# vocdoni/gnark-crypto-primitives

Hardware: AMD Instinct MI355X
Metric: proofs/sec, Arbo-160 Poseidon SMT-verifier circuit, Groth16/BN254 (higher is better)
Workload: dtype u32x8 Montgomery (254-bit integer)

## Files before the change

### gnark_crypto_primitives_amd/csrc/api.hip

```cpp
#include <algorithm>

#include "zkmi_internal.h"
#include "ff29.h"
#include "ec29.h"

using namespace zk;

namespace zk {

int ensure_scratch(zkmi_ctx* ctx, DevBuf& s, size_t bytes, void** out) {
  if (s.bytes < bytes) {
    if (s.p) {
      hipStreamSynchronize(ctx->stream);
      if (ctx->stream2) hipStreamSynchronize(ctx->stream2);
      if (ctx->stream3) hipStreamSynchronize(ctx->stream3);
      hipFree(s.p);
      s.p = nullptr;
      s.bytes = 0;
    }
    hipError_t e = hipMalloc(&s.p, bytes);
    if (e != hipSuccess) {
      ctx->err = "hipMalloc(" + std::to_string(bytes) + " B) failed: " + hipGetErrorString(e) +
                 " (the working set of this batch does not fit beside the MSM tables: load the key"
                 " with zkmi_pk_desc.max_batch >= the batch size, or with a table_budget_bytes cap)";
      s.p = nullptr;
      return ZKMI_ERR_OOM;
    }
    s.bytes = bytes;
  }
  if (out) *out = s.p;
  return ZKMI_OK;
}

int require_idle(zkmi_ctx* ctx) {
  if (!ctx->sets[0].pending && !ctx->sets[1].pending) return ZKMI_OK;
// ... 559 lines not shown
int zkmi_msm_bases_load(zkmi_ctx* ctx, int group, const void* bases, size_t n, int window_bits,
                        zkmi_msm_bases** out) {
  return zkmi_msm_bases_load_image(ctx, group, bases, n, window_bits, 0, out);
}

int zkmi_msm_bases_load_image(zkmi_ctx* ctx, int group, const void* bases, size_t n,
                              int window_bits, int image, zkmi_msm_bases** out) {
  ZK_HIP(hipSetDevice(ctx->device));
  if (!out) return ZKMI_ERR_ARG;
  if (image != 0 && image != 1) {
    ctx->err = "image must be 0 (x * 2^256) or 1 (x * 2^261)";
    return ZKMI_ERR_ARG;
  }
  if (!window_bits_ok(window_bits)) {
    ctx->err = "window_bits must be 0 (auto), in [2,16], 100 + [4,16], 200 + [2,20] or 300 + [3,21]";
    return ZKMI_ERR_ARG;
  }
  Staged sb(ctx);
  int rc = sb.in(bases, n * (group == 1 ? 64 : 128));
  if (rc) return rc;
  WinPlan plan;
  if (window_bits) {
    plan = plan_explicit(window_bits);
  } else {
    const double usable = usable_table_bytes_standalone(n);
    plan = plan_windows_for_budget(n, group, (group == 1 ? 0.64 : 0.34) * usable);
    int c1, c2;
    plan_shared_for_budget(group == 1 ? n : 0, group == 2 ? n : 0, 0.9 * usable, &c1, &c2);
    const WinPlan ps = plan_shared(group == 1 ? c1 : c2);
    if (ps.W < plan.W) plan = ps;
    if (n >= 64) {
      int k1, k2;
      bool s1, s2;
      plan_comb_for_budget(group == 1 ? n : 0, group == 2 ? n : 0, 0.9 * usable, &k1, &k2, &s1, &s2);
      const int k = group == 1 ? k1 : k2;
      if ((double)COMB_W / k < (double)plan.W) plan = plan_comb(k, group == 1 ? s1 : s2);
    }
  }
  return bases_load_plan(ctx, group, sb.dev, n, plan, window_bits == 0, out,
                         image ? MSM_IMAGE_F : MSM_IMAGE_STD);
}

void zkmi_msm_bases_free(zkmi_ctx* ctx, zkmi_msm_bases* b) {
  if (!b) return;
  if (ctx) {
    hipSetDevice(ctx->device);
    hipStreamSynchronize(ctx->stream);
  }
  if (b->table) hipFree(b->table);
  if (b->inf) hipFree(b->inf);
  delete b;
}

uint32_t zkmi_comb_min_groups_per_chunk(void) { return COMB_MIN_GROUPS_PER_CHUNK; }

int zkmi_msm_batch(zkmi_ctx* ctx, const zkmi_msm_bases* bases, const void* scalars, size_t batch,
                   void* out) {
  ZK_HIP(hipSetDevice(ctx->device));
  int rc;
  if ((rc = require_idle(ctx))) return rc;
  if (batch == 0) return ZKMI_OK;
  const size_t n = bases->n, Bp = round_up(batch, 64);
  const size_t pt = bases->group == 1 ? 64 : 128;
  Staged ss(ctx), so(ctx);
  if ((rc = ss.in(scalars, batch * n * 32)) || (rc = so.out(out, batch * pt))) return rc;
  void *sbi, *acc, *aff;
  if ((rc = ensure_scratch(ctx, ctx->sets[0].a, (n ? n : 1) * Bp * 32, &sbi)) ||
// ... 106 lines not shown
  zkmi_msm_bases_free(ctx, pk->B1);
  zkmi_msm_bases_free(ctx, pk->K);
  zkmi_msm_bases_free(ctx, pk->Z);
  zkmi_msm_bases_free(ctx, pk->B2);
  zkmi_msm_bases_free(ctx, pk->D1);
  zkmi_msm_bases_free(ctx, pk->D2);
  commit_keys_free(ctx, pk);
  if (pk->idx3) hipFree(pk->idx3);
  if (pk->a_wire) hipFree(pk->a_wire);
  if (pk->b_wire) hipFree(pk->b_wire);
  if (pk->k_wire) hipFree(pk->k_wire);
  delete pk;
}

static int wires_from_infinity(zkmi_ctx* ctx, const uint8_t* inf, uint32_t n_wires, uint32_t want,
                               const char* name, std::vector<uint32_t>* out) {
  std::vector<uint8_t> host(n_wires);
  if (n_wires && hipMemcpy(host.data(), inf, n_wires, hipMemcpyDefault) != hipSuccess) {
    ctx->err = std::string("pk: cannot read ") + name;
    return ZKMI_ERR_HIP;
  }
  out->clear();
  for (uint32_t i = 0; i < n_wires; i++)
    if (!host[i]) out->push_back(i);
  if (out->size() != want) {
    ctx->err = std::string("pk: ") + name + " retains " + std::to_string(out->size()) +
               " wires but the key holds " + std::to_string(want) + " points";
    return ZKMI_ERR_ARG;
  }
  return ZKMI_OK;
}

int zkmi_pk_load(zkmi_ctx* ctx, const zkmi_pk_desc* d, zkmi_pk** out) {
  ZK_HIP(hipSetDevice(ctx->device));
  if (!d || !out) return ZKMI_ERR_ARG;
  if (d->log_n < 1 || d->log_n > 28) {
    ctx->err = "pk: log_n out of range [1,28]";
    return ZKMI_ERR_ARG;
  }
  if (d->n_z + 1 < (1u << d->log_n)) {
    ctx->err = "pk: n_z must be at least 2^log_n - 1";
    return ZKMI_ERR_ARG;
  }
  const uint32_t n_z = (1u << d->log_n) - 1;
  std::vector<uint32_t> wa, wb, wk;
  {
    int rc;
    struct { const uint32_t* p; uint32_t n; const char* name; std::vector<uint32_t>* v; } idx[3] = {
        {d->a_wire, d->n_a, "a_wire", &wa}, {d->b_wire, d->n_b, "b_wire", &wb},
        {d->k_wire, d->n_k, "k_wire", &wk}};
    for (auto& t : idx) {
      if (!t.p) continue;
      t.v->resize(t.n);
      if (t.n && hipMemcpy(t.v->data(), t.p, (size_t)t.n * 4, hipMemcpyDefault) != hipSuccess) {
        ctx->err = std::string("pk: cannot read ") + t.name;
        return ZKMI_ERR_HIP;
      }
    }
    if (!d->a_wire) {
      if (!d->infinity_a) {
        ctx->err = "pk: neither a_wire nor infinity_a given";
        return ZKMI_ERR_ARG;
      }
      if ((rc = wires_from_infinity(ctx, d->infinity_a, d->n_wires, d->n_a, "infinity_a", &wa)))
        return rc;
    }
    if (!d->b_wire) {
      if (!d->infinity_b) {
// ... 56 lines not shown
  pk->log_n = d->log_n;
  pk->n_wires = d->n_wires;
  pk->n_a = d->n_a;
  pk->n_b = d->n_b;
  pk->n_k = n_kb;
  pk->n_z = n_zb;
  pk->folded = fold.folded;
  pk->fold_n_constraints = fold.folded ? d->fold_r1cs->n_constraints : 0;
  pk->max_batch = d->max_batch ? d->max_batch : 1024;
  int rc;
  if ((rc = commit_keys_load(ctx, d, pk))) {
    zkmi_pk_free(ctx, pk);
    return rc;
  }
  const bool auto1 = d->window_bits_g1 == 0, auto2 = d->window_bits_g2 == 0;
  const size_t n1 = (size_t)d->n_a + d->n_b + n_kb + n_zb;
  const size_t n_msm_max = std::max(std::max((size_t)d->n_a, (size_t)d->n_b),
                                    std::max((size_t)n_kb, (size_t)n_zb));
  const size_t n_slots = d->n_slots_hint ? d->n_slots_hint : (size_t)d->n_wires + d->n_wires / 20;
  const double ws = prove_working_set_bytes(d->log_n, n_slots, d->n_wires, pk->max_batch, n_msm_max,
                                            pk->commits.size());
  double usable = free_hbm_bytes() - ws;
  if (usable < 0) usable = 0;
  if (d->table_budget_bytes && (double)d->table_budget_bytes < usable)
    usable = (double)d->table_budget_bytes;
  int sc1 = 0, sc2 = 0;
  plan_shared_for_budget(n1, d->n_b, 0.98 * usable, &sc1, &sc2);
  WinPlan p1 = auto1 ? plan_windows_for_budget(n1, 1, 0.64 * usable)
                     : plan_explicit((int)d->window_bits_g1);
  WinPlan p2 = auto2 ? plan_windows_for_budget(d->n_b, 2, 0.34 * usable)
                     : plan_explicit((int)d->window_bits_g2);
  if (auto1 && sc1 && plan_shared(sc1).W < p1.W) p1 = plan_shared(sc1);
  if (auto2 && sc2 && plan_shared(sc2).W < p2.W) p2 = plan_shared(sc2);
  if (n1 >= 4096) {
    int k1 = 0, k2 = 0;
    bool s1 = true, s2 = true;
    plan_comb_for_budget(auto1 ? n1 : 0, auto2 ? d->n_b : 0, 0.98 * usable, &k1, &k2, &s1, &s2,
                         d->sparse_witness == 0);
    if (auto1 && (double)COMB_W / k1 < (double)p1.W) p1 = plan_comb(k1, s1);
    if (auto2 && (double)COMB_W / k2 < (double)p2.W) p2 = plan_comb(k2, s2);
  }
  WinPlan p1z = p1;
  if (d->sparse_witness >= 2 && auto1 && auto2 && n1 >= 4096 && n_zb >= 4096) {
    const int kw = 12;
    const double wire_bytes =
        (double)((d->n_a + kw - 1) / kw + (d->n_b + kw - 1) / kw + (n_kb + kw - 1) / kw) *
            (double)(1u << kw) * 64.0 +
        (double)((d->n_b + kw - 1) / kw) * (double)(1u << kw) * 128.0;
    if (wire_bytes < 0.5 * usable) {
      int kz = 0, k2 = 0;
      bool sz = true, s2 = true;
      plan_comb_for_budget(n_zb, 0, 0.98 * usable - wire_bytes, &kz, &k2, &sz, &s2, true);
      p1 = plan_comb(kw, false);
      p2 = plan_comb(kw, false);
      p1z = plan_comb(kz, sz);
    }
  }
  auto load = [&](int group, const void* pts, size_t n, const WinPlan& plan, bool relax,
                  zkmi_msm_bases** out, int image) -> int {
    Staged sb(ctx);
    int r = sb.in(pts, n * (group == 1 ? 64 : 128));
    if (r) return r;
    r = bases_load_plan(ctx, group, sb.dev, n, plan, relax, out, image);
    if (!r) (*out)->chunk_factor = d->msm_chunk_factor;
    return r;
  };
  if ((rc = upload_u32(ctx, wa.data(), d->n_a, &pk->a_wire)) ||
      (rc = upload_u32(ctx, wb.data(), d->n_b, &pk->b_wire)) ||
      (rc = upload_u32(ctx, fold.folded ? fold.k_wire.data() : wk.data(), n_kb, &pk->k_wire)) ||
      (rc = load(1, d->g1_a, d->n_a, p1, auto1, &pk->A, MSM_IMAGE_F)) ||
      (rc = load(1, d->g1_b, d->n_b, p1, auto1, &pk->B1, MSM_IMAGE_F)) ||
      (rc = load(1, fold.folded ? (const void*)fold.k.data() : d->g1_k, n_kb, p1, auto1, &pk->K,
                 MSM_IMAGE_F)) ||
      (rc = load(1, fold.folded ? (const void*)fold.e.data() : d->g1_z, n_zb, p1z, auto1, &pk->Z,
                 MSM_IMAGE_STD)) ||
      (rc = load(2, d->g2_b, d->n_b, p2, auto2, &pk->B2, MSM_IMAGE_F))) {
    zkmi_pk_free(ctx, pk);
    return rc;
  }
  {
    const uint32_t idx[3] = {0, 1, 2};
    if ((rc = upload_u32(ctx, idx, 3, &pk->idx3)) ||
        (rc = zkmi_msm_bases_load(ctx, 1, d->g1_delta, 1, 8, &pk->D1)) ||
        (rc = zkmi_msm_bases_load(ctx, 2, d->g2_delta, 1, 8, &pk->D2))) {
      zkmi_pk_free(ctx, pk);
      return rc;
    }
    pk->D1->side = pk->D2->side = 2;
  }
  hipMemcpy(&pk->alpha, d->g1_alpha, 64, hipMemcpyDefault);
  hipMemcpy(&pk->beta1, d->g1_beta, 64, hipMemcpyDefault);
  hipMemcpy(&pk->delta1, d->g1_delta, 64, hipMemcpyDefault);
  hipMemcpy(&pk->beta2, d->g2_beta, 128, hipMemcpyDefault);
  hipMemcpy(&pk->delta2, d->g2_delta, 128, hipMemcpyDefault);
  *out = pk;
  return ZKMI_OK;
}

int zkmi_pk_info(const zkmi_pk* pk, uint64_t* info) {
  if (!pk || !info) return ZKMI_ERR_ARG;
  info[0] = (uint64_t)pk->Z->plan.W;
  info[1] = pk->Z->plan.per_base;
  info[2] = (uint64_t)pk->B2->plan.W;
  info[3] = pk->B2->plan.per_base;
  info[4] = pk->A->table_bytes + pk->B1->table_bytes + pk->K->table_bytes + pk->Z->table_bytes;
  info[5] = pk->B2->table_bytes;
  info[6] = pk->Z->plan.shared;
  info[7] = pk->B2->plan.shared;
  info[8] = pk->Z->plan.comb;
  info[9] = pk->B2->plan.comb;
  return ZKMI_OK;
}

int zkmi_pk_folded(const zkmi_pk* pk) { return pk && pk->folded ? 1 : 0; }

void zkmi_cs_free(zkmi_ctx* ctx, zkmi_cs* cs) {
  if (!cs) return;
  if (ctx) hipSetDevice(ctx->device);
  if (cs->program) hipFree(cs->program);
  if (cs->consts) hipFree(cs->consts);
  delete cs;
}

int zkmi_cs_load(zkmi_ctx* ctx, const zkmi_cs_desc* d, zkmi_cs** out) {
  ZK_HIP(hipSetDevice(ctx->device));
  if (!d || !out) return ZKMI_ERR_ARG;
  auto* cs = new zkmi_cs();
  const std::string err =
      vprog_validate({d->n_wires, d->n_slots, d->n_consts, d->n_constraints, d->n_rows,
                      d->lanes_per_proof},
                     d->program, &cs->commit_rows, &cs->has_emul);
  if (!err.empty()) {
    delete cs;
    ctx->err = err;
    return ZKMI_ERR_ARG;
  }
  cs->n_wires = d->n_wires;
  cs->n_public = d->n_public;
  cs->n_secret = d->n_secret;
  cs->n_constraints = d->n_constraints;
  cs->n_slots = d->n_slots;
  cs->n_rows = d->n_rows;
  cs->n_consts = d->n_consts;
// ... 215 lines not shown
}

int zkmi_prove_collect(zkmi_ctx* ctx, void* proofs_out, int32_t* status_out) {
  return zkmi_prove_collect_ex(ctx, proofs_out, status_out, nullptr);
}

int zkmi_prove_collect_ex(zkmi_ctx* ctx, void* proofs_out, int32_t* status_out,
                          void* commitments_out) {
  ZK_HIP(hipSetDevice(ctx->device));
  const int si = ctx->next_collect;
  zkmi_ctx::ProveSet& S = ctx->sets[si];
  if (!S.pending) {
    ctx->err = "prove: nothing submitted";
    return ZKMI_ERR_ARG;
  }
  if (!S.pk->commits.empty() && !commitments_out) {
    ctx->err = "prove: this key has commitments: collect with zkmi_prove_collect_ex";
    return ZKMI_ERR_ARG;
  }
  const zkmi_pk* pk = S.pk;
  const size_t batch = S.batch, Bp = S.Bp;
  int rc;
  if (!S.heavy_enqueued && (rc = enqueue_heavy(ctx, si))) return rc;
  SumsView v(S.sums.p, Bp);
  hipStream_t q3 = ctx->stream3;
  ZK_HIP(hipStreamWaitEvent(q3, S.evq[4], 0));
  hipEventRecord(S.eva[0], q3);
  if (pk->Z->plan.shared || pk->Z->plan.comb) {
    void* ws[4] = {v.w1[0], v.w1[1], v.w1[2], v.w1[3]};
    void* os[4] = {v.sA, v.sB1, v.sK, v.sZ};
    const zkmi_msm_bases* ms[4] = {pk->A, pk->B1, pk->K, pk->Z};
    bool same = true;
    for (int i = 0; i < 3; i++)
      same = same && ms[i]->plan.bits[0] == pk->Z->plan.bits[0] &&
             ms[i]->plan.comb == pk->Z->plan.comb &&
             ms[i]->plan.comb_signed == pk->Z->plan.comb_signed;
    if (same) {
      if ((rc = msm_horner_run(ctx, q3, 4, ms, ws, os, Bp))) return rc;
    } else {
      for (int i = 0; i < 4; i++)
        if ((rc = msm_horner_run(ctx, q3, 1, ms + i, ws + i, os + i, Bp))) return rc;
    }
  }
  if (pk->B2->plan.shared || pk->B2->plan.comb) {
    void* ws[1] = {v.w2};
    void* os[1] = {v.sB2};
    const zkmi_msm_bases* ms[1] = {pk->B2};
    if ((rc = msm_horner_run(ctx, q3, 1, ms, ws, os, Bp))) return rc;
  }
  PkConsts pc{pk->alpha, pk->beta1, pk->beta2};
  hipLaunchKernelGGL(assemble_kernel, dim3((unsigned)(Bp / 64)), dim3(64), 0, q3, v.sA, v.sB1, v.sK,
                     v.sZ, v.tR, v.tS, v.tNRS, (const Fr*)S.rs, Bp, pc, v.proofs);
  hipLaunchKernelGGL(assemble_g2_kernel, dim3((unsigned)(Bp / 64)), dim3(64), 0, q3, v.sB2, v.tS2,
                     Bp, pk->beta2, v.proofs);
  ZK_HIP(hipGetLastError());
  ZK_HIP(hipMemcpyAsync(proofs_out, v.proofs, batch * 256, hipMemcpyDefault, q3));
  ZK_HIP(hipMemcpyAsync(status_out, S.st, batch * 4, hipMemcpyDefault, q3));
  if (const size_t nc = pk->commits.size()) {
    const size_t pitch = (nc + 1) * 64;
    for (size_t i = 0; i < nc; i++)
      ZK_HIP(hipMemcpy2DAsync((char*)commitments_out + i * 64, pitch,
                              (const char*)S.commit_pts + i * Bp * 64, 64, 64, batch, hipMemcpyDefault, q3));
    ZK_HIP(hipMemcpy2DAsync((char*)commitments_out + nc * 64, pitch,
                            (const char*)S.commit_pok + Bp * 128, 64, 64, batch, hipMemcpyDefault, q3));
  }
  hipEventRecord(S.eva[1], q3);
  zkmi_ctx::ProveSet& N = ctx->sets[si ^ 1];
  if (N.pending && !N.heavy_enqueued && (rc = enqueue_heavy(ctx, si ^ 1))) return rc;
  ZK_HIP(hipEventSynchronize(S.eva[1]));
// ... 37 lines not shown
```

### gnark_crypto_primitives_amd/csrc/msm.hip

```cpp
#include "msm_impl.h"

namespace zk {

WinPlan plan_with_windows(int W) {
  WinPlan p;
  if (W < 16) W = 16;
  if (W > 64) W = 64;
  p.W = W;
  const int c0 = 255 / W, rem = 255 - c0 * W;
  uint32_t off = 0;
  for (int j = 0; j < W; j++) {
    p.bits[j] = (uint8_t)(j < rem ? c0 + 1 : c0);
    p.off[j] = off;
    off += 1u << (p.bits[j] - 1);
  }
  p.per_base = off;
  return p;
}
WinPlan plan_uniform(int c) {
  WinPlan p;
  p.W = (255 + c - 1) / c;
  uint32_t off = 0;
  for (int j = 0; j < p.W; j++) {
    p.bits[j] = (uint8_t)c;
    p.off[j] = off;
    off += 1u << (c - 1);
  }
  p.per_base = off;
  return p;
}
WinPlan plan_shared(int c) {
  WinPlan p;
  if (c < 4) c = 4;
  if (c > 16) c = 16;
  p.shared = 1;
  p.W = (255 + c - 1) / c;
  for (int j = 0; j < p.W; j++) {
    p.bits[j] = (uint8_t)(j + 1 < p.W ? c : 255 - (p.W - 1) * c);
    p.off[j] = 0;
  }
  p.per_base = 1u << (c - 1);
  return p;
}
WinPlan plan_comb(int k, bool signed_tables) {
  WinPlan p;
  if (k < 2) k = 2;
  if (k > 21) k = 21;
  if (!signed_tables && k > 20) k = 20;
  p.comb = (uint8_t)k;
  p.comb_signed = signed_tables ? 1 : 0;
  p.W = COMB_W + (signed_tables ? 1 : 0);
  p.per_base = 0;
  return p;
}
void plan_comb_for_budget(size_t n1, size_t n2, double usable_bytes, int* k1, int* k2, bool* sg1,
                          bool* sg2, bool allow_signed) {
  double best = 1e300;
  *k1 = *k2 = 8;
  *sg1 = *sg2 = allow_signed;
  for (int s1 = 0; s1 < (allow_signed ? 2 : 1); s1++)
    for (int s2 = 0; s2 < (allow_signed ? 2 : 1); s2++)
      for (int a = 8; a <= (s1 ? 21 : 20); a++)
        for (int b = 8; b <= (s2 ? 21 : 20); b++) {
          const double g1 = (double)((n1 + a - 1) / a), g2 = (double)((n2 + b - 1) / b);
          const double bytes = g1 * (double)(1u << (a - s1)) * 64.0 + g2 * (double)(1u << (b - s2)) * 128.0;
          if (bytes > usable_bytes) continue;
          const double cost = g1 * (s1 ? 255 * 62.8 : 254 * 61.1) + g2 * (s2 ? 255 * 178.5 : 254 * 171.6);
          if (cost < best) {
            best = cost;
            *k1 = a;
            *k2 = b;
            *sg1 = s1 != 0;
            *sg2 = s2 != 0;
          }
        }
}
void plan_shared_for_budget(size_t n1, size_t n2, double usable_bytes, int* c1, int* c2) {
  double best = 1e300;
  *c1 = *c2 = 4;
  for (int a = 4; a <= 16; a++)
    for (int b = 4; b <= 16; b++) {
      const double bytes = (double)n1 * (1u << (a - 1)) * 64.0 + (double)n2 * (1u << (b - 1)) * 128.0;
      if (bytes > usable_bytes) continue;
      const double cost = (double)n1 * ((255 + a - 1) / a) + 3.0 * (double)n2 * ((255 + b - 1) / b);
      if (cost < best) {
        best = cost;
        *c1 = a;
        *c2 = b;
      }
    }
}
WinPlan plan_windows_for_budget(size_t n_total, int group, double budget_bytes) {
  const double entry = group == 1 ? 64.0 : 128.0;
  for (int W = 16; W <= 64; W++) {
    WinPlan p = plan_with_windows(W);
    if ((double)n_total * p.per_base * entry <= budget_bytes) return p;
  }
  return plan_with_windows(64);
}

extern template int build_comb<Fq2>(zkmi_ctx*, const Affine<Fq2>*, size_t, const WinPlan&, int,
                                    Affine<Fq2>*, int*, Affine<Fq2>*);
extern template int build_impl<Fq2>(zkmi_ctx*, const Affine<Fq2>*, size_t, const WinPlan&,
                                    Affine<Fq2>*);
extern template int run_impl<Fq2>(zkmi_ctx*, const zkmi_msm_bases*, const Fr*, const uint32_t*,
                                  size_t, size_t, XYZZ<Fq2>*, bool, XYZZ<Fq2>*, hipStream_t,
                                  const uint8_t*, bool);

// ... 130 lines not shown
```

### gnark_crypto_primitives_amd/groth16.py

```python
from __future__ import annotations

import ctypes as C
import random

import numpy as np

from . import lib as _lib
from .frontend.compile import CompiledCircuit, R, ints_to_array, to_mont_array

P = 21888242871839275222246405745257275088696311157297823662689037894645226208583
_MONT_P = (1 << 256) % P

G1_GEN = (1, 2)
G2_GEN = ((10857046999023057135944570762232829481370756359578518086990519993285655852781,
           11559732032986387107991004021392285783925812861821192530917403151452391805634),
          (8495653923123431417604973247489272438418190587263600148770280649306958101930,
           4082367875863433681332203403145435568316851327593401208105741076214120093531))


def _fq_mont(xs):
    return ints_to_array([x % P * _MONT_P % P for x in xs])


def g1_gen_mont():
# ... 126 lines not shown
    vk.g2_beta, vk.g2_delta, vk.g2_gamma = pk.g2_beta, pk.g2_delta, g2_pts[nb + 2].copy()
    return pk, vk, trapdoor


def commit_fn(pk: ProvingKey):
    from . import hash_to_field, verify as _v
    bases = [[_v.g1_from_image(b) for b in ck["basis"]] for ck in pk.commitment_keys]

    def fn(idx, hashed, committed):
        acc = None
        for pt, s in zip(bases[idx], committed):
            if s % R and pt is not None:
                acc = _v._g1_add(acc, _v._g1_mul(pt, s % R))
        return hash_to_field.commitment_challenge(acc, hashed)
    return fn


def gpu_mul(ctx: _lib.Context):
    def mul(group, scalars):
        n = scalars.shape[0]
        out = np.zeros((n, 8 if group == 1 else 16), dtype=np.uint64)
        if n:
            ctx.fixed_base_mul(group, g1_gen_mont() if group == 1 else g2_gen_mont(), scalars, n,
                               out)
        return out
    return mul


class Prover:

    def __init__(self, ctx: _lib.Context, cc: CompiledCircuit, pk: ProvingKey,
                 window_bits_g1: int = 0, window_bits_g2: int = 0, *, max_batch: int = 0,
                 table_budget_bytes: int = 0, msm_chunk_factor: int = 0,
                 gnark_key_layout: bool = False, sparse_witness=None, fold_quotient=None):
        self.ctx, self.cc, self.pk = ctx, cc, pk
        self.n_inputs = cc.n_inputs
        self._consts = to_mont_array(cc.consts) if cc.consts else np.zeros((0, 4), np.uint64)
        prog = self._prog = np.ascontiguousarray(cc.vprogram, dtype=np.uint32)
        cd = _lib.CsDesc(cc.n_wires, cc.n_public, cc.n_secret, cc.n_constraints, cc.v_n_slots,
                         cc.v_n_rows, len(cc.consts), cc.lanes_per_proof, prog.ctypes.data,
                         self._consts.ctypes.data)
        self.cs_h = ctx.cs_load(cd)
        self._keep = [np.ascontiguousarray(x) for x in
                      (pk.a_wire, pk.b_wire, pk.k_wire, pk.g1_a, pk.g1_b, pk.g1_k, pk.g1_z, pk.g2_b,
                       pk.g1_alpha, pk.g1_beta, pk.g1_delta, pk.g2_beta, pk.g2_delta)]
        k = self._keep
        ptrs = [x.ctypes.data for x in k]
        inf_a = inf_b = None
        n_public = 0
        if gnark_key_layout:
            inf_a, inf_b = pk.infinity_maps()
            self._keep += [inf_a, inf_b]
            ptrs[0] = ptrs[1] = ptrs[2] = None
            n_public = cc.n_public
        self.n_commitments = len(pk.commitment_keys)
        cdescs = (_lib.CommitmentDesc * max(self.n_commitments, 1))()
        for i, ck in enumerate(pk.commitment_keys):
            arrs = [np.ascontiguousarray(ck["private"], dtype=np.uint32),
                    np.ascontiguousarray(ck["hashed"], dtype=np.uint32),
                    np.ascontiguousarray(ck["basis"], dtype=np.uint64),
                    np.ascontiguousarray(ck["basis_exp_sigma"], dtype=np.uint64)]
            self._keep += arrs
            cdescs[i] = _lib.CommitmentDesc(len(ck["private"]), len(ck["hashed"]), ck["wire"], 0,
                                            *[a.ctypes.data for a in arrs])
        self._keep.append(cdescs)
        if len(getattr(cc, "commitments", [])) != self.n_commitments:
            raise ValueError("circuit and proving key disagree on the number of commitments")
        fold = None
        if fold_quotient is None:
            fold_quotient = not self.n_commitments
        if fold_quotient and cc.consts and cc.n_constraints:
            fold, fold_keep = self._r1cs_desc()
            self._keep += fold_keep + [fold]
        pd = _lib.PkDesc(pk.log_n, pk.n_wires, len(pk.a_wire), len(pk.b_wire), len(pk.k_wire),
                         pk.g1_z.shape[0], *ptrs, window_bits_g1, window_bits_g2,
                         inf_a.ctypes.data if inf_a is not None else None,
                         inf_b.ctypes.data if inf_b is not None else None, n_public,
                         max_batch, table_budget_bytes, cc.v_n_slots, msm_chunk_factor,
                         (2 if cc.n_boolean_wires * 100 >= cc.n_wires * 99 else
                          int(cc.n_boolean_wires * 2 > cc.n_wires)) if sparse_witness is None
                         else int(sparse_witness),
                         self.n_commitments,
                         C.addressof(cdescs) if self.n_commitments else None,
                         C.addressof(fold) if fold is not None else None)
        self.pk_h = ctx.pk_load(pd)
        self.folded = ctx.pk_folded(self.pk_h)

    def _r1cs_desc(self):
        cc = self.cc
        coeffs = to_mont_array(cc.consts)
        keep = [coeffs]
        fields = []
        for ptr, col, cid in (cc.L, cc.Rm, cc.O):
            terms = np.ascontiguousarray(np.stack([cid, col], axis=1).astype(np.uint32))
            ptr = np.ascontiguousarray(ptr, dtype=np.uint32)
            keep += [ptr, terms]
            fields += [ptr.ctypes.data, terms.ctypes.data]
        return (_lib.R1csDesc(cc.n_wires, cc.n_constraints, len(cc.consts), coeffs.ctypes.data,
                              *fields), keep)

    def load_r1cs(self):
        if getattr(self, "r1cs_h", None):
            return self.r1cs_h
        rd, _keep = self._r1cs_desc()
        self.r1cs_h = self.ctx.r1cs_load(rd)
        return self.r1cs_h

    def load_r1cs_solver(self, lanes_per_proof=0, hints="basic"):
        sets = {"basic": _lib.HINTS_BASIC, "std": _lib.HINTS_STD}
        if hints not in sets:
            raise ValueError('hints must be "basic" or "std"')
        if getattr(self, "r1cs_solver_h", None):
            if (lanes_per_proof, hints) == self._r1cs_solver_args:
                return self.r1cs_solver_h
            self.ctx.r1cs_solver_free(self.r1cs_solver_h)
            self.r1cs_solver_h = None
        cc = self.cc
        kinds, in_ptr, lc_ptr, hcol, hcid, out_ptr, outs = cc.hint_arrays
# ... 135 lines not shown
```

### gnark_crypto_primitives_amd/lib.py

```python
from __future__ import annotations

import ctypes as C
import os

import numpy as np

_HERE = os.path.dirname(os.path.abspath(__file__))
LIB_PATH = os.environ.get("ZKMI_LIB", os.path.join(_HERE, "libzkmi.so"))

ZKMI_OK = 0
ZKMI_ERR_UNSATISFIED = -5


class ZkmiError(RuntimeError):
    pass


class PkDesc(C.Structure):
    _fields_ = [("log_n", C.c_uint32), ("n_wires", C.c_uint32), ("n_a", C.c_uint32),
                ("n_b", C.c_uint32), ("n_k", C.c_uint32), ("n_z", C.c_uint32),
                ("a_wire", C.c_void_p), ("b_wire", C.c_void_p), ("k_wire", C.c_void_p),
                ("g1_a", C.c_void_p), ("g1_b", C.c_void_p), ("g1_k", C.c_void_p),
                ("g1_z", C.c_void_p), ("g2_b", C.c_void_p), ("g1_alpha", C.c_void_p),
                ("g1_beta", C.c_void_p), ("g1_delta", C.c_void_p), ("g2_beta", C.c_void_p),
# ... 31 lines not shown
    _fields_ = [("n_public", C.c_uint32), ("n_secret", C.c_uint32), ("n_instr", C.c_uint32),
                ("n_hints", C.c_uint32), ("instr", C.c_void_p), ("hint_kind", C.c_void_p),
                ("hint_in_ptr", C.c_void_p), ("hint_lc_ptr", C.c_void_p), ("hint_terms", C.c_void_p),
                ("hint_out_ptr", C.c_void_p), ("hint_out", C.c_void_p),
                ("lanes_per_proof", C.c_uint32), ("hint_set", C.c_uint32)]


HINTS_BASIC, HINTS_STD = 0, 1


_P, _SZ, _I = C.c_void_p, C.c_size_t, C.c_int
SYMBOLS = [
    ("zkmi_init", _I, [_I, C.POINTER(_P)]),
    ("zkmi_destroy", None, [_P]),
    ("zkmi_last_error", C.c_char_p, [_P]),
    ("zkmi_sync", _I, [_P]),
    ("zkmi_stream", _P, [_P]),
    ("zkmi_field_mul", _I, [_P, _I, _P, _P, _P, _SZ]),
    ("zkmi_ff29_op", _I, [_P, _I, _I, _P, _P, _SZ]),
    ("zkmi_field_mul_bench", _I, [_P, _I, _SZ, _I, C.POINTER(C.c_double)]),
    ("zkmi_ntt_batch", _I, [_P, _P, _I, _SZ, _I, _I]),
    ("zkmi_h_batch", _I, [_P, _P, _P, _P, _P, _I, _SZ]),
    ("zkmi_ab_coset_batch", _I, [_P, _P, _P, _P, _I, _SZ]),
    ("zkmi_quotient_bases", _I, [_P, _P, _SZ, _I, _P, _P]),
    ("zkmi_msm_bases_load", _I, [_P, _I, _P, _SZ, _I, C.POINTER(_P)]),
    ("zkmi_msm_bases_free", None, [_P, _P]),
    ("zkmi_msm_batch", _I, [_P, _P, _P, _SZ, _P]),
    ("zkmi_msm_bases_load_image", _I, [_P, _I, _P, _SZ, _I, _I, C.POINTER(_P)]),
    ("zkmi_msm_batch_rows", _I, [_P, _P, _P, _SZ, _P, _SZ, _I, _I, _P]),
    ("zkmi_comb_min_groups_per_chunk", C.c_uint32, []),
    ("zkmi_fixed_base_mul", _I, [_P, _I, _P, _P, _SZ, _P]),
    ("zkmi_pk_load", _I, [_P, C.POINTER(PkDesc), C.POINTER(_P)]),
    ("zkmi_pk_free", None, [_P, _P]),
    ("zkmi_pk_info", _I, [_P, C.POINTER(C.c_uint64)]),
    ("zkmi_pk_folded", _I, [_P]),
    ("zkmi_cs_load", _I, [_P, C.POINTER(CsDesc), C.POINTER(_P)]),
    ("zkmi_cs_free", None, [_P, _P]),
    ("zkmi_solve_batch", _I, [_P, _P, _P, _SZ, _P, _P, _P]),
    ("zkmi_prove_batch", _I, [_P, _P, _P, _P, _SZ, _P, _P, _P]),
    ("zkmi_prove_submit", _I, [_P, _P, _P, _P, _SZ, _P]),
    ("zkmi_prove_collect", _I, [_P, _P, _P]),
    ("zkmi_prove_collect_ex", _I, [_P, _P, _P, _P]),
    ("zkmi_prove_witness_batch", _I, [_P, _P, _P, _P, _P, _P, _SZ, _SZ, _P, _P]),
    ("zkmi_host_alloc", _P, [_P, _SZ]),
    ("zkmi_host_free", None, [_P, _P]),
    ("zkmi_set_copy_threads", _I, [_P, _I]),
    ("zkmi_r1cs_load", _I, [_P, C.POINTER(R1csDesc), C.POINTER(_P)]),
    ("zkmi_r1cs_free", None, [_P, _P]),
    ("zkmi_prove_witness_submit", _I, [_P, _P, _P, _P, _P, _P, _P, _SZ, _SZ, _P]),
    ("zkmi_r1cs_solver_load", _I, [_P, _P, C.POINTER(R1csSolverDesc), C.POINTER(_P)]),
    ("zkmi_r1cs_solver_free", None, [_P, _P]),
    ("zkmi_r1cs_solver_info", _I, [_P, C.POINTER(C.c_uint64)]),
    ("zkmi_r1cs_solve_batch", _I, [_P, _P, _P, _SZ, _P, _P, _P]),
    ("zkmi_prove_r1cs_submit", _I, [_P, _P, _P, _P, _SZ, _P]),
    ("zkmi_last_timings", _I, [_P, C.POINTER(C.c_double)]),
    ("zkmi_plonk_pk_load", _I, [_P, _P, C.POINTER(_P)]),
    ("zkmi_plonk_pk_free", None, [_P, _P]),
    ("zkmi_plonk_round1", _I, [_P, _P, _P, _P, _SZ, _P, _P, _P]),
    ("zkmi_plonk_round2", _I, [_P, _P, _P, _P]),
    ("zkmi_plonk_round3", _I, [_P, _P, _P, _P]),
    ("zkmi_plonk_round4", _I, [_P, _P, _P, _P]),
    ("zkmi_plonk_round5", _I, [_P, _P, _P, _P]),
    ("zkmi_plonk_prove", _I, [_P, _P, _P, _P, _SZ, _P, _P, _P, _P]),
]

_lib = None

# ... 109 lines not shown
        self._check(self.lib.zkmi_msm_bases_load(self.h, group, _ptr(bases), n, window_bits,
                                                 C.byref(h)), "zkmi_msm_bases_load")
        return h

    def msm_bases_free(self, h):
        self.lib.zkmi_msm_bases_free(self.h, h)

    def msm_batch(self, bases_h, scalars, batch, out):
        self._check(self.lib.zkmi_msm_batch(self.h, bases_h, _ptr(scalars), batch, _ptr(out)),
                    "zkmi_msm_batch")
        return out

    def msm_bases_load_image(self, group, bases, n, window_bits, image):
        h = C.c_void_p()
        self._check(self.lib.zkmi_msm_bases_load_image(self.h, group, _ptr(bases), n, window_bits,
                                                       image, C.byref(h)),
                    "zkmi_msm_bases_load_image")
        return h

    def msm_batch_rows(self, bases_h, scalars, n_rows, row_idx, batch, image, uniform, out):
        self._check(self.lib.zkmi_msm_batch_rows(self.h, bases_h, _ptr(scalars), n_rows,
                                                 _ptr(row_idx), batch, image, uniform, _ptr(out)),
                    "zkmi_msm_batch_rows")
        return out

    def comb_min_groups_per_chunk(self):
        return int(self.lib.zkmi_comb_min_groups_per_chunk())

    def fixed_base_mul(self, group, base, scalars, n, out):
        self._check(self.lib.zkmi_fixed_base_mul(self.h, group, _ptr(base), _ptr(scalars), n,
                                                 _ptr(out)), "zkmi_fixed_base_mul")
        return out

    def pk_load(self, desc: PkDesc):
        h = C.c_void_p()
        self._check(self.lib.zkmi_pk_load(self.h, C.byref(desc), C.byref(h)), "zkmi_pk_load")
        return h

    def pk_info(self, h):
        arr = (C.c_uint64 * 10)()
        self._check(self.lib.zkmi_pk_info(h, arr), "zkmi_pk_info")
        return dict(zip(("g1_windows", "g1_entries_per_base", "g2_windows", "g2_entries_per_base",
                         "g1_table_bytes", "g2_table_bytes", "g1_shared", "g2_shared",
                         "g1_comb_k", "g2_comb_k"), [int(x) for x in arr]))

    def pk_folded(self, h) -> bool:
        return bool(self.lib.zkmi_pk_folded(h))

    def pk_free(self, h):
        self.lib.zkmi_pk_free(self.h, h)

    def cs_load(self, desc: CsDesc):
        h = C.c_void_p()
        self._check(self.lib.zkmi_cs_load(self.h, C.byref(desc), C.byref(h)), "zkmi_cs_load")
        return h

    def cs_free(self, h):
        self.lib.zkmi_cs_free(self.h, h)

    def solve_batch(self, cs_h, inputs, batch, wires_out=None, abc_out=None, status_out=None):
        if status_out is None:
            status_out = np.zeros(batch, dtype=np.int32)
        self._check(self.lib.zkmi_solve_batch(self.h, cs_h, _ptr(inputs), batch, _ptr(wires_out),
                                              _ptr(abc_out), _ptr(status_out)), "zkmi_solve_batch")
        return status_out

    def prove_batch(self, pk_h, cs_h, inputs, batch, rs, proofs_out, status_out):
        self._check(self.lib.zkmi_prove_batch(self.h, pk_h, cs_h, _ptr(inputs), batch, _ptr(rs),
                                              _ptr(proofs_out), _ptr(status_out)),
                    "zkmi_prove_batch")

    def prove_submit(self, pk_h, cs_h, inputs, batch, rs):
        self._check(self.lib.zkmi_prove_submit(self.h, pk_h, cs_h, _ptr(inputs), batch, _ptr(rs)),
                    "zkmi_prove_submit")

    def prove_collect(self, proofs_out, status_out, commitments_out=None):
        if commitments_out is None:
# ... 78 lines not shown
```

### include/zkmi.h

```cpp
#ifndef ZKMI_H
#define ZKMI_H
#include <stddef.h>
#include <stdint.h>

#ifdef __cplusplus
extern "C" {
#endif

typedef struct zkmi_ctx zkmi_ctx;
typedef struct zkmi_pk zkmi_pk;
typedef struct zkmi_cs zkmi_cs;
typedef struct zkmi_r1cs_desc zkmi_r1cs_desc;

enum zkmi_status {
  ZKMI_OK = 0,
  ZKMI_ERR_ARG = -1,
  ZKMI_ERR_HIP = -2,
  ZKMI_ERR_NO_DEVICE = -3,
  ZKMI_ERR_OOM = -4,
  ZKMI_ERR_UNSATISFIED = -5
};

int zkmi_init(int device, zkmi_ctx** out);
void zkmi_destroy(zkmi_ctx* ctx);
// ... 42 lines not shown

typedef struct {
  uint32_t log_n;
  uint32_t n_wires;
  uint32_t n_a, n_b, n_k, n_z;
  const uint32_t* a_wire;
  const uint32_t* b_wire;
  const uint32_t* k_wire;
  const void* g1_a;
  const void* g1_b;
  const void* g1_k;
  const void* g1_z;
  const void* g2_b;
  const void* g1_alpha;
  const void* g1_beta;
  const void* g1_delta;
  const void* g2_beta;
  const void* g2_delta;
  uint32_t window_bits_g1;
  uint32_t window_bits_g2;
  const uint8_t* infinity_a;
  const uint8_t* infinity_b;
  uint32_t n_public;
  uint32_t max_batch;
  uint64_t table_budget_bytes;
  uint32_t n_slots_hint;
  uint32_t msm_chunk_factor;
  uint32_t sparse_witness;
  uint32_t n_commitments;
  const zkmi_commitment_desc* commitments;
  const zkmi_r1cs_desc* fold_r1cs;
} zkmi_pk_desc;
int zkmi_pk_load(zkmi_ctx* ctx, const zkmi_pk_desc* desc, zkmi_pk** out);
void zkmi_pk_free(zkmi_ctx* ctx, zkmi_pk* pk);
int zkmi_pk_info(const zkmi_pk* pk, uint64_t* info );
int zkmi_pk_folded(const zkmi_pk* pk);

typedef struct {
  uint32_t n_wires, n_public, n_secret, n_constraints;
  uint32_t n_slots, n_rows, n_consts;
  uint32_t lanes_per_proof;
  const uint32_t* program;
  const void* consts;
} zkmi_cs_desc;
int zkmi_cs_load(zkmi_ctx* ctx, const zkmi_cs_desc* desc, zkmi_cs** out);
void zkmi_cs_free(zkmi_ctx* ctx, zkmi_cs* cs);

int zkmi_solve_batch(zkmi_ctx* ctx, const zkmi_cs* cs, const void* inputs, size_t batch,
                     void* wires_out, void* abc_out, int32_t* status_out);

int zkmi_prove_batch(zkmi_ctx* ctx, const zkmi_pk* pk, const zkmi_cs* cs, const void* inputs,
                     size_t batch, const void* rs, void* proofs_out, int32_t* status_out);

int zkmi_prove_submit(zkmi_ctx* ctx, const zkmi_pk* pk, const zkmi_cs* cs, const void* inputs,
                      size_t batch, const void* rs);
int zkmi_prove_collect(zkmi_ctx* ctx, void* proofs_out, int32_t* status_out);
int zkmi_prove_collect_ex(zkmi_ctx* ctx, void* proofs_out, int32_t* status_out,
                          void* commitments_out);

void* zkmi_host_alloc(zkmi_ctx* ctx, size_t bytes);
void zkmi_host_free(zkmi_ctx* ctx, void* p);
int zkmi_set_copy_threads(zkmi_ctx* ctx, int threads);

typedef struct {
  uint32_t coeff;
  uint32_t wire;
} zkmi_term;
struct zkmi_r1cs_desc {
// ... 94 lines not shown
```

Measured before the change: 8615.

## Search per-MSM comb table sizes under memory budget instead of one shared size

Replaces the single comb window size shared by the A, B1, K and Z G1 MSMs with a branch-and-bound search that picks a comb width and signedness for each of the five MSMs. The search weights the Z MSM more heavily than the others and bounds the total cost to stay near the equal-size plan. The Horner batching check is relaxed so that MSMs with different comb widths can still run together. An explicit per-MSM override API and a plan-query API are also added. The aim is to give more of the table memory budget to the MSMs where it lowers the most group additions. The risk is an uneven split that slows the A, B1 and K MSMs, or breaks the batched Horner path.

```diff
diff --git a/gnark_crypto_primitives_amd/csrc/api.hip b/gnark_crypto_primitives_amd/csrc/api.hip
--- a/gnark_crypto_primitives_amd/csrc/api.hip
+++ b/gnark_crypto_primitives_amd/csrc/api.hip
@@ -1,6 +1,7 @@
 #include <algorithm>
 
 #include "zkmi_internal.h"
+#include "comb_plan.h"
 #include "ff29.h"
 #include "ec29.h"
 
@@ -626,7 +627,7 @@
     if (n >= 64) {
       int k1, k2;
       bool s1, s2;
-      plan_comb_for_budget(group == 1 ? n : 0, group == 2 ? n : 0, 0.9 * usable, &k1, &k2, &s1, &s2);
+      comb_plan_equal(group == 1 ? n : 0, group == 2 ? n : 0, 0.9 * usable, &k1, &k2, &s1, &s2, true);
       const int k = group == 1 ? k1 : k2;
       if ((double)COMB_W / k < (double)plan.W) plan = plan_comb(k, group == 1 ? s1 : s2);
     }
@@ -799,8 +800,25 @@
 }
 
 int zkmi_pk_load(zkmi_ctx* ctx, const zkmi_pk_desc* d, zkmi_pk** out) {
+  return zkmi_pk_load_planned(ctx, d, nullptr, out);
+}
+
+int zkmi_pk_load_planned(zkmi_ctx* ctx, const zkmi_pk_desc* d, const uint32_t* msm_window_bits,
+                         zkmi_pk** out) {
   ZK_HIP(hipSetDevice(ctx->device));
   if (!d || !out) return ZKMI_ERR_ARG;
+  if (msm_window_bits)
+    for (int i = 0; i < COMB_PLAN_MSMS; i++)
+      if (msm_window_bits[i] == 0 || !window_bits_ok((int)msm_window_bits[i])) {
+        ctx->err = "pk: msm_window_bits must be in [2,16], 100 + [4,16], 200 + [2,20] or 300 + [3,21]";
+        return ZKMI_ERR_ARG;
+      }
+  if (msm_window_bits)
+    for (int i = 0; i < COMB_MSM_Z; i++)
+      if ((msm_window_bits[i] >= 100) != (msm_window_bits[COMB_MSM_Z] >= 100)) {
+        ctx->err = "pk: msm_window_bits of A, B1, K and Z must all be per-window plans or none";
+        return ZKMI_ERR_ARG;
+      }
   if (d->log_n < 1 || d->log_n > 28) {
     ctx->err = "pk: log_n out of range [1,28]";
     return ZKMI_ERR_ARG;
@@ -923,15 +941,18 @@
                      : plan_explicit((int)d->window_bits_g2);
   if (auto1 && sc1 && plan_shared(sc1).W < p1.W) p1 = plan_shared(sc1);
   if (auto2 && sc2 && plan_shared(sc2).W < p2.W) p2 = plan_shared(sc2);
+  WinPlan pm[COMB_PLAN_MSMS] = {p1, p1, p1, p1, p2};
   if (n1 >= 4096) {
-    int k1 = 0, k2 = 0;
-    bool s1 = true, s2 = true;
-    plan_comb_for_budget(auto1 ? n1 : 0, auto2 ? d->n_b : 0, 0.98 * usable, &k1, &k2, &s1, &s2,
-                         d->sparse_witness == 0);
-    if (auto1 && (double)COMB_W / k1 < (double)p1.W) p1 = plan_comb(k1, s1);
-    if (auto2 && (double)COMB_W / k2 < (double)p2.W) p2 = plan_comb(k2, s2);
-  }
-  WinPlan p1z = p1;
+    const size_t nm[COMB_PLAN_MSMS] = {auto1 ? d->n_a : 0u, auto1 ? d->n_b : 0u, auto1 ? n_kb : 0u,
+                                       auto1 ? n_zb : 0u, auto2 ? d->n_b : 0u};
+    const CombPlan eq = comb_plan_equal5(nm, 0.98 * usable, d->sparse_witness == 0);
+    const CombPlan cp = comb_plan_search(nm, 0.98 * usable, d->sparse_witness == 0);
+    for (int i = 0; i < COMB_PLAN_MSMS; i++) {
+      const bool g2 = comb_msm_is_g2(i);
+      if ((g2 ? auto2 : auto1) && (double)COMB_W / eq.k[i] < (double)(g2 ? p2 : p1).W)
+        pm[i] = plan_comb(cp.k[i], cp.sg[i]);
+    }
+  }
   if (d->sparse_witness >= 2 && auto1 && auto2 && n1 >= 4096 && n_zb >= 4096) {
     const int kw = 12;
     const double wire_bytes =
@@ -941,12 +962,17 @@
     if (wire_bytes < 0.5 * usable) {
       int kz = 0, k2 = 0;
       bool sz = true, s2 = true;
-      plan_comb_for_budget(n_zb, 0, 0.98 * usable - wire_bytes, &kz, &k2, &sz, &s2, true);
-      p1 = plan_comb(kw, false);
-      p2 = plan_comb(kw, false);
-      p1z = plan_comb(kz, sz);
-    }
-  }
+      comb_plan_equal(n_zb, 0, 0.98 * usable - wire_bytes, &kz, &k2, &sz, &s2, true);
+      for (int i = 0; i < COMB_PLAN_MSMS; i++) pm[i] = plan_comb(kw, false);
+      pm[COMB_MSM_Z] = plan_comb(kz, sz);
+    }
+  }
+  bool relax[COMB_PLAN_MSMS] = {auto1, auto1, auto1, auto1, auto2};
+  if (msm_window_bits)
+    for (int i = 0; i < COMB_PLAN_MSMS; i++) {
+      pm[i] = plan_explicit((int)msm_window_bits[i]);
+      relax[i] = false;
+    }
   auto load = [&](int group, const void* pts, size_t n, const WinPlan& plan, bool relax,
                   zkmi_msm_bases** out, int image) -> int {
     Staged sb(ctx);
@@ -959,13 +985,13 @@
   if ((rc = upload_u32(ctx, wa.data(), d->n_a, &pk->a_wire)) ||
       (rc = upload_u32(ctx, wb.data(), d->n_b, &pk->b_wire)) ||
       (rc = upload_u32(ctx, fold.folded ? fold.k_wire.data() : wk.data(), n_kb, &pk->k_wire)) ||
-      (rc = load(1, d->g1_a, d->n_a, p1, auto1, &pk->A, MSM_IMAGE_F)) ||
-      (rc = load(1, d->g1_b, d->n_b, p1, auto1, &pk->B1, MSM_IMAGE_F)) ||
-      (rc = load(1, fold.folded ? (const void*)fold.k.data() : d->g1_k, n_kb, p1, auto1, &pk->K,
-                 MSM_IMAGE_F)) ||
-      (rc = load(1, fold.folded ? (const void*)fold.e.data() : d->g1_z, n_zb, p1z, auto1, &pk->Z,
-                 MSM_IMAGE_STD)) ||
-      (rc = load(2, d->g2_b, d->n_b, p2, auto2, &pk->B2, MSM_IMAGE_F))) {
+      (rc = load(1, d->g1_a, d->n_a, pm[COMB_MSM_A], relax[COMB_MSM_A], &pk->A, MSM_IMAGE_F)) ||
+      (rc = load(1, d->g1_b, d->n_b, pm[COMB_MSM_B1], relax[COMB_MSM_B1], &pk->B1, MSM_IMAGE_F)) ||
+      (rc = load(1, fold.folded ? (const void*)fold.k.data() : d->g1_k, n_kb, pm[COMB_MSM_K],
+                 relax[COMB_MSM_K], &pk->K, MSM_IMAGE_F)) ||
+      (rc = load(1, fold.folded ? (const void*)fold.e.data() : d->g1_z, n_zb, pm[COMB_MSM_Z],
+                 relax[COMB_MSM_Z], &pk->Z, MSM_IMAGE_STD)) ||
+      (rc = load(2, d->g2_b, d->n_b, pm[COMB_MSM_B2], relax[COMB_MSM_B2], &pk->B2, MSM_IMAGE_F))) {
     zkmi_pk_free(ctx, pk);
     return rc;
   }
@@ -1000,6 +1026,16 @@
   info[7] = pk->B2->plan.shared;
   info[8] = pk->Z->plan.comb;
   info[9] = pk->B2->plan.comb;
+  return ZKMI_OK;
+}
+
+int zkmi_pk_msm_plan(const zkmi_pk* pk, uint32_t* plan) {
+  if (!pk || !plan) return ZKMI_ERR_ARG;
+  const zkmi_msm_bases* ms[COMB_PLAN_MSMS] = {pk->A, pk->B1, pk->K, pk->Z, pk->B2};
+  for (int i = 0; i < COMB_PLAN_MSMS; i++) {
+    plan[i] = ms[i]->plan.comb;
+    plan[COMB_PLAN_MSMS + i] = ms[i]->plan.comb_signed;
+  }
   return ZKMI_OK;
 }
 
@@ -1281,9 +1317,9 @@
     const zkmi_msm_bases* ms[4] = {pk->A, pk->B1, pk->K, pk->Z};
     bool same = true;
     for (int i = 0; i < 3; i++)
-      same = same && ms[i]->plan.bits[0] == pk->Z->plan.bits[0] &&
-             ms[i]->plan.comb == pk->Z->plan.comb &&
-             ms[i]->plan.comb_signed == pk->Z->plan.comb_signed;
+      same = same && (ms[i]->plan.comb != 0) == (pk->Z->plan.comb != 0) &&
+             ms[i]->plan.comb_signed == pk->Z->plan.comb_signed &&
+             (pk->Z->plan.comb || (ms[i]->plan.shared && ms[i]->plan.bits[0] == pk->Z->plan.bits[0]));
     if (same) {
       if ((rc = msm_horner_run(ctx, q3, 4, ms, ws, os, Bp))) return rc;
     } else {
diff --git a/gnark_crypto_primitives_amd/csrc/comb_plan.h b/gnark_crypto_primitives_amd/csrc/comb_plan.h
--- /dev/null
+++ b/gnark_crypto_primitives_amd/csrc/comb_plan.h
@@ -0,0 +1,161 @@
+#pragma once
+#include <cstddef>
+#include <cstdint>
+
+namespace zk {
+
+constexpr int COMB_PLAN_MSMS = 5;
+enum { COMB_MSM_A = 0, COMB_MSM_B1 = 1, COMB_MSM_K = 2, COMB_MSM_Z = 3, COMB_MSM_B2 = 4 };
+constexpr int COMB_PLAN_MIN_K = 8;
+constexpr int COMB_PLAN_MAX_K_SIGNED = 21;
+constexpr int COMB_PLAN_MAX_K_UNSIGNED = 20;
+constexpr double COMB_PLAN_PHI = 0.5;
+constexpr double COMB_PLAN_GUARD = 0.02;
+
+struct CombPlan {
+  int k[COMB_PLAN_MSMS];
+  bool sg[COMB_PLAN_MSMS];
+  bool fits;
+};
+
+inline bool comb_msm_is_g2(int i) { return i == COMB_MSM_B2; }
+inline double comb_groups(size_t n, int k) { return (double)((n + (size_t)k - 1) / (size_t)k); }
+inline double comb_group_cost(bool g2, bool sg) {
+  return g2 ? (sg ? 255 * 178.5 : 254 * 171.6) : (sg ? 255 * 62.8 : 254 * 61.1);
+}
+inline double comb_table_bytes(size_t n, bool g2, int k, bool sg) {
+  return comb_groups(n, k) * (double)((uint64_t)1 << (k - (sg ? 1 : 0))) * (g2 ? 128.0 : 64.0);
+}
+inline double comb_plan_bytes(const size_t n[COMB_PLAN_MSMS], const CombPlan& p) {
+  double b = 0;
+  for (int i = 0; i < COMB_PLAN_MSMS; i++) b += comb_table_bytes(n[i], comb_msm_is_g2(i), p.k[i], p.sg[i]);
+  return b;
+}
+inline double comb_plan_cost(const size_t n[COMB_PLAN_MSMS], const CombPlan& p, double phi) {
+  double c = 0;
+  for (int i = 0; i < COMB_PLAN_MSMS; i++)
+    c += (i == COMB_MSM_Z ? 1.0 : phi) * comb_group_cost(comb_msm_is_g2(i), p.sg[i]) *
+         comb_groups(n[i], p.k[i]);
+  return c;
+}
+
+inline void comb_plan_equal(size_t n1, size_t n2, double usable_bytes, int* k1, int* k2, bool* sg1,
+                            bool* sg2, bool allow_signed) {
+  double best = 1e300;
+  *k1 = *k2 = COMB_PLAN_MIN_K;
+  *sg1 = *sg2 = allow_signed;
+  for (int s1 = 0; s1 < (allow_signed ? 2 : 1); s1++)
+    for (int s2 = 0; s2 < (allow_signed ? 2 : 1); s2++)
+      for (int a = COMB_PLAN_MIN_K; a <= (s1 ? COMB_PLAN_MAX_K_SIGNED : COMB_PLAN_MAX_K_UNSIGNED); a++)
+        for (int b = COMB_PLAN_MIN_K; b <= (s2 ? COMB_PLAN_MAX_K_SIGNED : COMB_PLAN_MAX_K_UNSIGNED); b++) {
+          const double bytes = comb_table_bytes(n1, false, a, s1 != 0) + comb_table_bytes(n2, true, b, s2 != 0);
+          if (bytes > usable_bytes) continue;
+          const double cost = comb_groups(n1, a) * comb_group_cost(false, s1 != 0) +
+                              comb_groups(n2, b) * comb_group_cost(true, s2 != 0);
+          if (cost < best) {
+            best = cost;
+            *k1 = a;
+            *k2 = b;
+            *sg1 = s1 != 0;
+            *sg2 = s2 != 0;
+          }
+        }
+}
+
+inline CombPlan comb_plan_equal5(const size_t n[COMB_PLAN_MSMS], double usable_bytes,
+                                 bool allow_signed) {
+  int k1, k2;
+  bool s1, s2;
+  comb_plan_equal(n[0] + n[1] + n[2] + n[3], n[4], usable_bytes, &k1, &k2, &s1, &s2, allow_signed);
+  CombPlan p;
+  for (int i = 0; i < COMB_PLAN_MSMS; i++) {
+    p.k[i] = comb_msm_is_g2(i) ? k2 : k1;
+    p.sg[i] = comb_msm_is_g2(i) ? s2 : s1;
+  }
+  p.fits = comb_plan_bytes(n, p) <= usable_bytes;
+  return p;
+}
+
+inline CombPlan comb_plan_search(const size_t n[COMB_PLAN_MSMS], double usable_bytes,
+                                 bool allow_signed, double phi = COMB_PLAN_PHI,
+                                 double guard = COMB_PLAN_GUARD) {
+  const CombPlan ref = comb_plan_equal5(n, usable_bytes, allow_signed);
+  const double worst_max = (1.0 + guard) * comb_plan_cost(n, ref, 1.0);
+  if (ref.fits && comb_plan_bytes(n, ref) < usable_bytes) usable_bytes = comb_plan_bytes(n, ref);
+  struct Opt {
+    int k;
+    bool sg;
+    double bytes, cost;
+  };
+  constexpr int MAX_OPTS = 2 * (COMB_PLAN_MAX_K_SIGNED - COMB_PLAN_MIN_K + 1);
+  Opt opts[COMB_PLAN_MSMS][MAX_OPTS];
+  int n_opts[COMB_PLAN_MSMS];
+  for (int i = 0; i < COMB_PLAN_MSMS; i++) {
+    const bool g2 = comb_msm_is_g2(i);
+    n_opts[i] = 0;
+    if (n[i] == 0) {
+      opts[i][n_opts[i]++] = {ref.k[i], ref.sg[i], 0.0, 0.0};
+      continue;
+    }
+    Opt all[MAX_OPTS];
+    int m = 0;
+    for (int s = 0; s < (allow_signed ? 2 : 1); s++)
+      for (int k = COMB_PLAN_MIN_K; k <= (s ? COMB_PLAN_MAX_K_SIGNED : COMB_PLAN_MAX_K_UNSIGNED); k++)
+        all[m++] = {k, s != 0, comb_table_bytes(n[i], g2, k, s != 0),
+                    comb_group_cost(g2, s != 0) * comb_groups(n[i], k)};
+    for (int a = 1; a < m; a++)
+      for (int b = a; b > 0 && (all[b].bytes < all[b - 1].bytes ||
+                                (all[b].bytes == all[b - 1].bytes && all[b].cost < all[b - 1].cost));
+           b--) {
+        const Opt t = all[b];
+        all[b] = all[b - 1];
+        all[b - 1] = t;
+      }
+    double least = 1e300;
+    for (int a = 0; a < m; a++)
+      if (all[a].cost < least) {
+        least = all[a].cost;
+        opts[i][n_opts[i]++] = all[a];
+      }
+  }
+  CombPlan best = ref;
+  double best_cost = 1e300, best_bytes = 1e300;
+  int c[COMB_PLAN_MSMS];
+  double bytes[COMB_PLAN_MSMS + 1], cost[COMB_PLAN_MSMS + 1], worst[COMB_PLAN_MSMS + 1];
+  bytes[0] = cost[0] = worst[0] = 0;
+  int d = 0;
+  c[0] = 0;
+  while (d >= 0) {
+    if (c[d] >= n_opts[d]) {
+      d--;
+      if (d >= 0) c[d]++;
+      continue;
+    }
+    const Opt& o = opts[d][c[d]];
+    bytes[d + 1] = bytes[d] + o.bytes;
+    if (bytes[d + 1] > usable_bytes) {
+      c[d] = n_opts[d];
+      continue;
+    }
+    cost[d + 1] = cost[d] + (d == COMB_MSM_Z ? 1.0 : phi) * o.cost;
+    worst[d + 1] = worst[d] + o.cost;
+    if (d + 1 < COMB_PLAN_MSMS) {
+      c[++d] = 0;
+      continue;
+    }
+    if (worst[d + 1] <= worst_max &&
+        (cost[d + 1] < best_cost || (cost[d + 1] == best_cost && bytes[d + 1] < best_bytes))) {
+      best_cost = cost[d + 1];
+      best_bytes = bytes[d + 1];
+      for (int i = 0; i < COMB_PLAN_MSMS; i++) {
+        best.k[i] = opts[i][c[i]].k;
+        best.sg[i] = opts[i][c[i]].sg;
+      }
+    }
+    c[d]++;
+  }
+  best.fits = best_cost < 1e300;
+  return best;
+}
+
+}
diff --git a/gnark_crypto_primitives_amd/csrc/msm.hip b/gnark_crypto_primitives_amd/csrc/msm.hip
--- a/gnark_crypto_primitives_amd/csrc/msm.hip
+++ b/gnark_crypto_primitives_amd/csrc/msm.hip
@@ -1,4 +1,5 @@
 #include "msm_impl.h"
+#include "comb_plan.h"
 
 namespace zk {
 
@@ -55,25 +56,7 @@
 }
 void plan_comb_for_budget(size_t n1, size_t n2, double usable_bytes, int* k1, int* k2, bool* sg1,
                           bool* sg2, bool allow_signed) {
-  double best = 1e300;
-  *k1 = *k2 = 8;
-  *sg1 = *sg2 = allow_signed;
-  for (int s1 = 0; s1 < (allow_signed ? 2 : 1); s1++)
-    for (int s2 = 0; s2 < (allow_signed ? 2 : 1); s2++)
-      for (int a = 8; a <= (s1 ? 21 : 20); a++)
-        for (int b = 8; b <= (s2 ? 21 : 20); b++) {
-          const double g1 = (double)((n1 + a - 1) / a), g2 = (double)((n2 + b - 1) / b);
-          const double bytes = g1 * (double)(1u << (a - s1)) * 64.0 + g2 * (double)(1u << (b - s2)) * 128.0;
-          if (bytes > usable_bytes) continue;
-          const double cost = g1 * (s1 ? 255 * 62.8 : 254 * 61.1) + g2 * (s2 ? 255 * 178.5 : 254 * 171.6);
-          if (cost < best) {
-            best = cost;
-            *k1 = a;
-            *k2 = b;
-            *sg1 = s1 != 0;
-            *sg2 = s2 != 0;
-          }
-        }
+  comb_plan_equal(n1, n2, usable_bytes, k1, k2, sg1, sg2, allow_signed);
 }
 void plan_shared_for_budget(size_t n1, size_t n2, double usable_bytes, int* c1, int* c2) {
   double best = 1e300;
diff --git a/gnark_crypto_primitives_amd/groth16.py b/gnark_crypto_primitives_amd/groth16.py
--- a/gnark_crypto_primitives_amd/groth16.py
+++ b/gnark_crypto_primitives_amd/groth16.py
@@ -182,7 +182,8 @@
     def __init__(self, ctx: _lib.Context, cc: CompiledCircuit, pk: ProvingKey,
                  window_bits_g1: int = 0, window_bits_g2: int = 0, *, max_batch: int = 0,
                  table_budget_bytes: int = 0, msm_chunk_factor: int = 0,
-                 gnark_key_layout: bool = False, sparse_witness=None, fold_quotient=None):
+                 gnark_key_layout: bool = False, sparse_witness=None, fold_quotient=None,
+                 msm_window_bits=None):
         self.ctx, self.cc, self.pk = ctx, cc, pk
         self.n_inputs = cc.n_inputs
         self._consts = to_mont_array(cc.consts) if cc.consts else np.zeros((0, 4), np.uint64)
@@ -233,7 +234,7 @@
                          self.n_commitments,
                          C.addressof(cdescs) if self.n_commitments else None,
                          C.addressof(fold) if fold is not None else None)
-        self.pk_h = ctx.pk_load(pd)
+        self.pk_h = ctx.pk_load(pd, msm_window_bits)
         self.folded = ctx.pk_folded(self.pk_h)
 
     def _r1cs_desc(self):
diff --git a/gnark_crypto_primitives_amd/lib.py b/gnark_crypto_primitives_amd/lib.py
--- a/gnark_crypto_primitives_amd/lib.py
+++ b/gnark_crypto_primitives_amd/lib.py
@@ -87,7 +87,9 @@
     ("zkmi_fixed_base_mul", _I, [_P, _I, _P, _P, _SZ, _P]),
     ("zkmi_pk_load", _I, [_P, C.POINTER(PkDesc), C.POINTER(_P)]),
     ("zkmi_pk_free", None, [_P, _P]),
+    ("zkmi_pk_load_planned", _I, [_P, C.POINTER(PkDesc), C.POINTER(C.c_uint32), C.POINTER(_P)]),
     ("zkmi_pk_info", _I, [_P, C.POINTER(C.c_uint64)]),
+    ("zkmi_pk_msm_plan", _I, [_P, C.POINTER(C.c_uint32)]),
     ("zkmi_pk_folded", _I, [_P]),
     ("zkmi_cs_load", _I, [_P, C.POINTER(CsDesc), C.POINTER(_P)]),
     ("zkmi_cs_free", None, [_P, _P]),
@@ -263,17 +265,27 @@
                                                  _ptr(out)), "zkmi_fixed_base_mul")
         return out
 
-    def pk_load(self, desc: PkDesc):
-        h = C.c_void_p()
-        self._check(self.lib.zkmi_pk_load(self.h, C.byref(desc), C.byref(h)), "zkmi_pk_load")
+    def pk_load(self, desc: PkDesc, msm_window_bits=None):
+        h = C.c_void_p()
+        if msm_window_bits is None:
+            self._check(self.lib.zkmi_pk_load(self.h, C.byref(desc), C.byref(h)), "zkmi_pk_load")
+        else:
+            wb = (C.c_uint32 * 5)(*msm_window_bits)
+            self._check(self.lib.zkmi_pk_load_planned(self.h, C.byref(desc), wb, C.byref(h)),
+                        "zkmi_pk_load_planned")
         return h
 
     def pk_info(self, h):
         arr = (C.c_uint64 * 10)()
         self._check(self.lib.zkmi_pk_info(h, arr), "zkmi_pk_info")
-        return dict(zip(("g1_windows", "g1_entries_per_base", "g2_windows", "g2_entries_per_base",
+        info = dict(zip(("g1_windows", "g1_entries_per_base", "g2_windows", "g2_entries_per_base",
                          "g1_table_bytes", "g2_table_bytes", "g1_shared", "g2_shared",
                          "g1_comb_k", "g2_comb_k"), [int(x) for x in arr]))
+        plan = (C.c_uint32 * 10)()
+        self._check(self.lib.zkmi_pk_msm_plan(h, plan), "zkmi_pk_msm_plan")
+        info["msm_comb_k"] = dict(zip(("A", "B1", "K", "Z", "B2"), [int(x) for x in plan[:5]]))
+        info["msm_comb_signed"] = dict(zip(("A", "B1", "K", "Z", "B2"), [int(x) for x in plan[5:]]))
+        return info
 
     def pk_folded(self, h) -> bool:
         return bool(self.lib.zkmi_pk_folded(h))
diff --git a/include/zkmi.h b/include/zkmi.h
--- a/include/zkmi.h
+++ b/include/zkmi.h
@@ -98,8 +98,11 @@
   const zkmi_r1cs_desc* fold_r1cs;
 } zkmi_pk_desc;
 int zkmi_pk_load(zkmi_ctx* ctx, const zkmi_pk_desc* desc, zkmi_pk** out);
+int zkmi_pk_load_planned(zkmi_ctx* ctx, const zkmi_pk_desc* desc, const uint32_t* msm_window_bits,
+                         zkmi_pk** out);
 void zkmi_pk_free(zkmi_ctx* ctx, zkmi_pk* pk);
 int zkmi_pk_info(const zkmi_pk* pk, uint64_t* info );
+int zkmi_pk_msm_plan(const zkmi_pk* pk, uint32_t* plan );
 int zkmi_pk_folded(const zkmi_pk* pk);
 
 typedef struct {
```

After: 8803 (median of 6 runs). +2.2%, better.
